# isl-org/Open3D

Hardware: AMD Instinct MI355X
Metric: RGB-D frames/s, TSDF integrate with known poses (configs[1]: touch + activate + integrate into an 8 mm / 16^3 VoxelBlockGrid); the ICP + integrate + ray-cast loop (configs[2]) is in loop_frames_per_s (its first tracked frame untimed as warm-up; the whole run in loop_frames_per_s_with_first_frame) (higher is better)
Workload: dtype f32; 1 GPU; block_count=50000, frames_per_launch=12, active_blocks=5745

## Files before the change

include/o3d_mi355x_host.h:

```cpp
#ifndef O3D_MI355X_HOST_H_
#define O3D_MI355X_HOST_H_

#include "o3d_mi355x.h"

#ifdef __cplusplus
extern "C" {
#endif

typedef struct {
    double relative_fitness;
    double relative_rmse;
    int max_iteration;
} o3dmi_icp_criteria_t;

typedef struct {
    double transformation[16];
    double inlier_rmse;
    double fitness;
    int converged;
    int num_iterations;
    int64_t num_correspondences;
} o3dmi_registration_result_t;

typedef void (*o3dmi_icp_callback_t)(int64_t iteration_index,
// ... 488 lines not shown
                          int frames_per_launch, int slice_rank,
                          int slice_world, void* segment_out_dev,
                          o3dmi_stream_t stream);
int o3dmi_vbg_integrate_frames_sliced(
        o3dmi_vbg_t* g, int n_frames, const void* const* depth_devs,
        int depth_rows, int depth_cols, const void* const* color_devs,
        int color_rows, int color_cols, int input_dtype,
        const double* depth_intrinsic, const double* color_intrinsic,
        const double* extrinsics, float depth_scale, float depth_max,
        float trunc_voxel_multiplier, int frames_per_launch,
        const void* const* gathered_devs, o3dmi_stream_t stream);
int o3dmi_vbg_sliced_stats(const o3dmi_vbg_t* g, int64_t* chunks,
                           int64_t* reapplied, int* capacity,
                           int* table_slots);

int o3dmi_vbg_profile_begin(o3dmi_vbg_t* g, int max_launches, int stride);
int o3dmi_vbg_profile_end(o3dmi_vbg_t* g, o3dmi_stream_t stream,
                          double* integrate_ms, int64_t* launches,
                          int64_t* block_frames, int64_t* frames);
int64_t o3dmi_vbg_profile_distinct_blocks(const o3dmi_vbg_t* g);
int o3dmi_vbg_division_forms(float voxel_size, float trunc_voxel_multiplier,
                             int wait);
int64_t o3dmi_vbg_step_form_launches(int form);
int64_t o3dmi_vbg_profile_launches(const o3dmi_vbg_t* g, int64_t capacity,
                                   float* ms, int32_t* block_frames,
                                   int32_t* distinct_blocks,
                                   int32_t* map_size);

int o3dmi_vbg_ray_cast(o3dmi_vbg_t* g, const int32_t* block_coords_dev,
                       int64_t m, const double* intrinsic,
                       const double* extrinsic, int width, int height,
                       float* range_map_dev, float* out_depth,
                       float* out_vertex, float* out_color, float* out_normal,
                       int64_t* out_index, uint8_t* out_mask, float* out_ratio,
                       float* out_ratio_dx, float* out_ratio_dy,
                       float* out_ratio_dz, float depth_scale, float depth_min,
                       float depth_max, float weight_threshold,
                       float trunc_voxel_multiplier, int range_map_down_factor,
                       o3dmi_stream_t stream);

int o3dmi_vbg_ray_cast_sharded(
        o3dmi_vbg_t* g, const int32_t* block_coords_dev, int64_t m,
        const double* intrinsic, const double* extrinsic, int width, int height,
        float* range_map_dev, float* out_depth, float* out_vertex,
        float* out_color, float* out_normal, float depth_scale, float depth_min,
        float depth_max, float weight_threshold, float trunc_voxel_multiplier,
// ... 153 lines not shown
```

open3d_amd/_lib.py:

```python
import ctypes as C
import os

_HERE = os.path.dirname(os.path.abspath(__file__))
SO_PATH = os.environ.get("O3DMI_LIB") or os.path.join(
    _HERE, "lib", "libo3d_mi355x.so")

OK = 0
F32, F64, U16, U8, I32, I64 = 0, 1, 2, 3, 4, 5
I8, I16, U32, U64, BOOL = 6, 7, 8, 9, 10

_vp = C.c_void_p
_i64 = C.c_int64
_i32 = C.c_int
_f = C.c_float
_d = C.c_double
_dp = C.POINTER(C.c_double)

PROTOTYPES = {
    "o3dmi_abi_version": (_i32, []),
    "o3dmi_status_string": (C.c_char_p, [_i32]),
    "o3dmi_last_error": (C.c_char_p, []),
    "o3dmi_device_info": (_i32, [C.c_char_p, C.c_size_t, C.POINTER(_i32),
                                 C.POINTER(_i64)]),
    "o3dmi_release_cached_memory": (_i32, []),
# ... 431 lines not shown
    "o3dmi_npz_get": (_i32, [_vp, C.c_char_p, C.POINTER(_i32),
                             C.POINTER(_i32), C.POINTER(_i64),
                             C.POINTER(_vp)]),
    "o3dmi_npz_write": (_i32, [_vp, C.c_char_p]),
    "o3dmi_npz_read": (_i32, [C.c_char_p, C.POINTER(_vp)]),
    "o3dmi_vbg_export_blocks": (_i32, [_vp, _i64, _vp, C.POINTER(_vp),
                                       C.POINTER(_i64), _vp]),
    "o3dmi_vbg_merge_blocks": (_i32, [_vp, _vp, C.POINTER(_vp), _i64, _vp]),
    "o3dmi_vbg_save": (_i32, [_vp, C.c_char_p, _vp]),
    "o3dmi_vbg_load": (_i32, [C.c_char_p, _vp, C.POINTER(_vp)]),
    "o3dmi_vbg_attribute_count": (_i32, [_vp]),
    "o3dmi_vbg_attribute_name": (C.c_char_p, [_vp, _i32]),
    "o3dmi_vbg_voxel_size": (_f, [_vp]),
    "o3dmi_vbg_block_resolution": (_i64, [_vp]),
    "o3dmi_vbg_ray_cast": (
        _i32, [_vp, _vp, _i64, _dp, _dp, _i32, _i32, _vp] + [_vp] * 10 +
        [_f, _f, _f, _f, _f, _i32, _vp]),
    "o3dmi_vbg_ray_cast_sharded": (
        _i32, [_vp, _vp, _i64, _dp, _dp, _i32, _i32, _vp] + [_vp] * 4 +
        [_f, _f, _f, _f, _f, _i32, _vp]),
    "o3dmi_vbg_profile_distinct_blocks": (_i64, [_vp]),
    "o3dmi_vbg_division_forms": (_i32, [_f, _f, _i32]),
    "o3dmi_vbg_step_form_launches": (_i64, [_i32]),
    "o3dmi_vbg_profile_launches": (_i64, [_vp, _i64, _vp, _vp, _vp, _vp]),
    "o3dmi_rccl_available": (_i32, []),
    "o3dmi_rccl_unique_id": (_i32, [_vp]),
    "o3dmi_comm_create_rccl": (_i32, [_vp, _i32, _i32, C.POINTER(_vp)]),
    "o3dmi_comm_adopt_rccl": (_i32, [_vp, C.POINTER(_vp)]),
    "o3dmi_comm_create_custom": (_i32, [_vp, _vp, _i32, _i32,
                                        C.POINTER(_vp)]),
    "o3dmi_comm_destroy": (_i32, [_vp]),
    "o3dmi_comm_rank": (_i32, [_vp]),
    "o3dmi_preload": (_i32, []),
    "o3dmi_comm_world": (_i32, [_vp]),
    "o3dmi_comm_rccl_ranks": (_i32, [_vp]),
    "o3dmi_set_comm": (_i32, [_vp]),
    "o3dmi_set_rccl_comm": (_i32, [_vp]),
    "o3dmi_comm_allreduce_sum_f64": (_i32, [_vp, _vp, _i64, _vp]),
    "o3dmi_comm_allgather": (_i32, [_vp, _vp, _vp, _i64, _vp]),
    "o3dmi_comm_alltoallv": (_i32, [_vp, _vp, C.POINTER(_i64),
                                    C.POINTER(_i64), _vp, C.POINTER(_i64),
                                    C.POINTER(_i64), _vp]),
    "o3dmi_vbg_merge_frame_sharded": (_i32, [_vp, _vp, _vp]),
    "o3dmi_vbg_allgather_owned_blocks": (_i32, [_vp, _vp, _vp]),
})

# ... 62 lines not shown
```

open3d_amd/csrc/common.h:

```cpp
#pragma once

#include <hip/hip_runtime.h>

#include <cstdint>
#include <cstdio>
#include <cstring>
#include <string>
#include <vector>

#include "o3d_mi355x.h"

namespace o3dmi {

void SetLastError(const std::string& msg);

int PoolAlloc(void** out, size_t bytes);
void PoolFree(void* p);

struct PoolScratch {
    hipStream_t s;
    std::vector<void*> blocks;
    explicit PoolScratch(hipStream_t st) : s(st) {}
    PoolScratch(const PoolScratch&) = delete;
    PoolScratch& operator=(const PoolScratch&) = delete;
// ... 250 lines not shown
                                   __HIP_MEMORY_SCOPE_AGENT) == in_class - 1) {
            __hip_atomic_store(&tickets[1 + cls], 0, __ATOMIC_RELAXED,
                               __HIP_MEMORY_SCOPE_AGENT);
            last = __hip_atomic_fetch_add(&tickets[0], 1, __ATOMIC_RELAXED,
                                          __HIP_MEMORY_SCOPE_AGENT) ==
                   classes - 1;
            if (last)
                __hip_atomic_store(&tickets[0], 0, __ATOMIC_RELAXED,
                                   __HIP_MEMORY_SCOPE_AGENT);
        }
        s_last_arrival = last;
    }
    __syncthreads();
    return s_last_arrival != 0;
}

constexpr int kTouchBits = 16;
__device__ __forceinline__ unsigned long long* TouchWord(const HashView& hv,
                                                         unsigned slot,
                                                         int plane) {
    return hv.slot_touch + ((size_t)plane * ((size_t)hv.mask + 1) + slot);
}
__device__ __forceinline__ bool TouchSlot(const HashView& hv, unsigned slot,
                                          unsigned long long stamp, int bit,
                                          int plane = 0) {
    unsigned long long* w = TouchWord(hv, slot, plane);
    unsigned long long cur = *w;
    while (true) {
        const bool fresh = (cur >> kTouchBits) != stamp;
        const unsigned long long want =
                fresh ? ((stamp << kTouchBits) | (1ull << bit))
                      : (cur | (1ull << bit));
        if (want == cur) return false;
        const unsigned long long old = atomicCAS(w, cur, want);
        if (old == cur) return fresh;
        cur = old;
    }
}


}

struct o3dmi_hash {
    o3dmi::HashView view;
    int64_t capacity = 0;
    int64_t n_slots = 0;
    int n_values = 0;
    int64_t value_dsizes[8] = {0};
    void* value_buffers[8] = {nullptr};
    int* scratch_count = nullptr;
    int* counters_host = nullptr;
};

namespace o3dmi {
int ClearHashAndCounter(o3dmi_hash* h, int* counter_dev, hipStream_t s);
// ... 2 lines not shown
```

open3d_amd/csrc/host/vbg_grid.cpp:

```cpp

#include <cstdlib>
#include <cstring>

#include "vbg.h"

using namespace o3dmi;

namespace {

int EnsureCapacity(o3dmi_vbg* g, int64_t length, o3dmi_stream_t stream) {
    if (g->size_event_pending) {
        O3DMI_HIP_CHECK(hipEventSynchronize(g->size_event));
        g->size_event_pending = false;
        g->size_bound = g->size_host[0];
    }
    int64_t capacity = o3dmi_hash_capacity(g->block_hashmap);
    if (g->size_bound + length <= capacity) {
        g->size_bound += length;
        return O3DMI_OK;
    }
    int64_t size = 0;
    int st = o3dmi_hash_size(g->block_hashmap, stream, &size);
    if (st) return st;
    int64_t new_size = size + length;
// ... 258 lines not shown
            e = hipHostMalloc((void**)&g->size_host, sizeof(int) * 4);
        if (e == hipSuccess)
            e = hipEventCreateWithFlags(&g->size_event, hipEventDisableTiming);
        if (e != hipSuccess) st = O3DMI_ERR_HIP;
    }
    if (st != O3DMI_OK) {
        o3dmi_vbg_destroy(g);
        return st;
    }
    if (block_resolution % 4 == 0)
        (void)PrefetchFastDivision(voxel_size * 8.0f, false);
    *out = g;
    return O3DMI_OK;
}

int o3dmi_vbg_division_forms(float voxel_size, float trunc_voxel_multiplier,
                             int wait) {
    return PrefetchFastDivision(voxel_size * trunc_voxel_multiplier, wait != 0);
}

int64_t o3dmi_vbg_step_form_launches(int form) {
    return (int64_t)StepFormLaunches(form);
}

int o3dmi_vbg_to_device(o3dmi_vbg_t* g, int device, o3dmi_vbg_t** out) {
    O3DMI_REQUIRE(g != nullptr && out != nullptr, "null argument");
    int cur = 0;
    O3DMI_HIP_CHECK(hipGetDevice(&cur));
    o3dmi_hash_t* hm = nullptr;
    int st = o3dmi_hash_to_device(g->block_hashmap, device, &hm);
    if (st) return st;
    auto* n = new o3dmi_vbg();
    n->voxel_size = g->voxel_size;
    n->block_resolution = g->block_resolution;
    n->attr_names = g->attr_names;
    n->attr_dtypes = g->attr_dtypes;
    n->attr_channels = g->attr_channels;
    n->owner_rank = g->owner_rank;
    n->owner_world = g->owner_world;
    n->block_hashmap = hm;
    hipError_t e = hipSetDevice(device);
    if (e == hipSuccess)
        e = hipMalloc((void**)&n->frame_count, sizeof(int32_t) * 4);
    if (e == hipSuccess)
        e = hipHostMalloc((void**)&n->size_host, sizeof(int) * 4);
    if (e == hipSuccess)
// ... 458 lines not shown
```

open3d_amd/csrc/stream_path.h:

```cpp
#pragma once

#include "common.h"

namespace o3dmi {

constexpr int kMaxGroup = 16;
static_assert(kMaxGroup == kTouchBits, "one touch bit per frame of a group");
constexpr int kDefaultGroup = 8;
constexpr int kGroupChunk = 4;

struct alignas(16) FrameBlock {
    int slot, x, y, z;
};

struct alignas(16) ReadyEntry {
    unsigned long long key;
    int block_idx;
    unsigned bits;
};

struct alignas(8) PixelRec {
    float d;
    unsigned rgba;
};
// ... 39 lines not shown
    int64_t list_capacity;
    int grid_hint;
    float* tsdf;
    void* weight;
    void* color;
    int grid_dtype;
    const double* depth_intrinsic;
    int resolution;
    float voxel_size, sdf_trunc, depth_max;
    float depth_scale;
    int* zero_counter;
    int* size_host;
    int status_stamp;
    int* prof_count;
    int* prof_frame_blocks;
    int* prof_map_size;
};

int LaunchFrameStep(o3dmi_hash* block_hash, const FrameFrontArgs* fronts,
                    int n_fronts, const IntegrateStreamArgs* integ,
                    hipStream_t s);

long long StepFormLaunches(int form);

int PrefetchFastDivision(float sdf_trunc, bool wait);

int RecoverOverflow(o3dmi_hash* block_hash, hipStream_t s, int64_t* wanted);

bool PrepTables(const double* depth_intrinsic, const double* color_intrinsic,
                int rows, int cols, int color_rows, int color_cols,
                float depth_scale, int* col, int* row);

int64_t FrustumBlockBound(const double* intrinsic, int rows, int cols,
                          float depth_max, float block_size, int stride);

}
```

open3d_amd/csrc/touch_device.h:

```cpp
#pragma once

#include "common.h"

namespace o3dmi {

template <bool kAllocate>
__device__ __forceinline__ bool InsertKey(const HashView& hv, int x, int y,
                                          int z, unsigned& slot_out,
                                          int overflow_stamp = 0) {
    slot_out = 0;
    if (kAllocate && overflow_stamp != 0 && hv.counters[3] != 0) return false;
    const int claim = ClaimSlot(hv, PackKey(x, y, z), slot_out,
                                !(kAllocate && overflow_stamp != 0));
    if (claim == -1 && kAllocate && overflow_stamp != 0) {
        atomicCAS(&hv.counters[3], 0, overflow_stamp);
        slot_out = 0;
        return false;
    }
    if (claim != 1) return false;
    if (kAllocate) {
        const unsigned h = slot_out;
        int top = atomicAdd(&hv.counters[0], 1);
        if (top >= hv.capacity) {
            if (overflow_stamp != 0) {
// ... 23 lines not shown
    int lane = threadIdx.x & 63;
    bool decided = !valid;
    while (remaining) {
        int first = __ffsll((long long)remaining) - 1;
        unsigned long long kf = __shfl(k, first);
        bool same = valid && (k == kf);
        unsigned long long same_mask = __ballot(same);
        if (same && !decided) {
            leader = (lane == first);
            decided = true;
        }
        remaining &= ~same_mask;
    }
    return leader;
}

struct TouchParams {
    Camera cam;
    int rows, cols, stride;
    int rows_strided, cols_strided;
    float block_size, sdf_trunc, depth_scale, depth_max;
};

template <typename depth_t>
__device__ __forceinline__ bool RayCandidates(const TouchParams& p,
                                              const depth_t* __restrict__ depth,
                                              int workload_idx, int (&xb)[4],
                                              int (&yb)[4], int (&zb)[4]) {
    int y = (workload_idx / p.cols_strided) * p.stride;
    int x = (workload_idx % p.cols_strided) * p.stride;
    float d = (float)depth[(int64_t)y * p.cols + x] / p.depth_scale;
    if (!(d > 0 && d < p.depth_max)) return false;

    float x_c, y_c, z_c, x_g, y_g, z_g;
    p.cam.Unproject((float)x, (float)y, 1.0f, x_c, y_c, z_c);
    p.cam.RigidTransform(x_c, y_c, z_c, x_g, y_g, z_g);
    float x_o = p.cam.e[0][3], y_o = p.cam.e[1][3], z_o = p.cam.e[2][3];
    float x_d = x_g - x_o, y_d = y_g - y_o, z_d = z_g - z_o;

    const float t_min = fmaxf(d - p.sdf_trunc, 0.0f);
    const float t_max = fminf(d + p.sdf_trunc, p.depth_max);
    const float t_step = (t_max - t_min) / 3;
    float t = t_min;
#pragma unroll
    for (int step = 0; step < 4; ++step) {
        xb[step] = (int)floorf((x_o + t * x_d) / p.block_size);
        yb[step] = (int)floorf((y_o + t * y_d) / p.block_size);
        zb[step] = (int)floorf((z_o + t * z_d) / p.block_size);
        t += t_step;
    }
    return true;
}


inline TouchParams MakeTouchParams(const double* intrinsic, const double* extrinsic,
                            int rows, int cols, int stride, int resolution,
                            float voxel_size, float sdf_trunc,
                            float depth_scale, float depth_max) {
    TouchParams p;
    double pose[16];
    InverseTransformation(extrinsic, pose);
    p.cam = Camera::Make(intrinsic, pose, 1.0f);
    p.rows = rows;
    p.cols = cols;
    p.stride = stride;
    p.rows_strided = rows / stride;
    p.cols_strided = cols / stride;
    p.block_size = voxel_size * resolution;
    p.sdf_trunc = sdf_trunc;
    p.depth_scale = depth_scale;
    p.depth_max = depth_max;
    return p;
}

// ... 3 lines not shown
```

open3d_amd/csrc/vbg_stream.hip:

```cpp

#include <cmath>

#include "common.h"
#include "preload.h"
#include <atomic>
#include <cmath>
#include <cstdio>
#include <cstdlib>
#include <cstring>
#include <map>
#include <mutex>
#include <string>
#include <type_traits>

#include "integrate_checks.h"
#include "stream_path.h"
#include "sliced_path.h"
#include "touch_device.h"

#ifndef O3DMI_ABLATE_GATHER
#define O3DMI_ABLATE_GATHER 0
#endif

namespace o3dmi {
namespace {

template <typename T, int N, int A>
struct alignas(A) Vec {
    T v[N];
};

__device__ __forceinline__ float DivByConst(float a, float b, float y) {
    const float q0 = a * y;
    const float r = __builtin_fmaf(-b, q0, a);
    return __builtin_fmaf(r, y, q0);
}
__device__ __forceinline__ float RecordDepth(float d, float depth_max) {
    return (!(d <= 0) && !(d > depth_max)) ? d : -__builtin_inff();
}

struct PrepParams {
    Camera color_cam;
    int color_rows, color_cols;
    bool with_color;
};

constexpr int kTileKeys = 2048;

struct FrontShared {
    TouchParams p;
    PrepParams pp;
    const int* col_lut;
    const int* row_lut;
    bool depth_div_short;
    bool prep_identity;
    float inv_depth_scale;
    FrameBlock* list;
    int64_t list_capacity;
    int* out_count;
    ReadyEntry* ready;
    int* tickets;
    int* touch_status;
    int n_touch_total;
    unsigned long long group_stamp;
    int touch_plane;
    int n_touch_wg, n_prep_wg;
};
inline bool SameIntrinsics(const Camera& a, const Camera& b) {
    return a.fx == b.fx && a.fy == b.fy && a.cx == b.cx && a.cy == b.cy &&
           a.scale == b.scale;
}
inline bool SameGroup(const FrontShared& a, const FrontShared& b) {
    return SameIntrinsics(a.p.cam, b.p.cam) && a.p.rows == b.p.rows &&
           a.p.cols == b.p.cols && a.p.stride == b.p.stride &&
           a.p.rows_strided == b.p.rows_strided &&
           a.p.cols_strided == b.p.cols_strided &&
           a.p.block_size == b.p.block_size &&
           a.p.sdf_trunc == b.p.sdf_trunc &&
           a.p.depth_scale == b.p.depth_scale &&
           a.p.depth_max == b.p.depth_max &&
           SameIntrinsics(a.pp.color_cam, b.pp.color_cam) &&
           a.pp.color_rows == b.pp.color_rows &&
           a.pp.color_cols == b.pp.color_cols &&
           a.pp.with_color == b.pp.with_color && a.col_lut == b.col_lut &&
           a.row_lut == b.row_lut && a.depth_div_short == b.depth_div_short &&
           a.prep_identity == b.prep_identity &&
           a.inv_depth_scale == b.inv_depth_scale && a.list == b.list &&
           a.list_capacity == b.list_capacity && a.out_count == b.out_count &&
           a.ready == b.ready && a.tickets == b.tickets &&
           a.touch_status == b.touch_status &&
           a.n_touch_total == b.n_touch_total &&
           a.group_stamp == b.group_stamp && a.touch_plane == b.touch_plane &&
           a.n_touch_wg == b.n_touch_wg && a.n_prep_wg == b.n_prep_wg;
}
struct FrontFrame {
    float pose[3][4];
    const uint16_t* depth;
    const uint8_t* color;
    PixelRec* recs;
    int group_bit;
};

struct FrontParams {
    TouchParams p;
    PrepParams pp;
    const uint16_t* depth;
    const uint8_t* color;
    const int* col_lut;
    const int* row_lut;
    bool depth_div_short;
    bool prep_identity;
    float inv_depth_scale;
    PixelRec* recs;
    FrameBlock* list;
    int64_t list_capacity;
    int* out_count;
    ReadyEntry* ready;
    int* tickets;
    int* touch_status;
    int n_touch_total;
    unsigned long long group_stamp;
    int group_bit;
    int touch_plane;
    int n_touch_wg, n_prep_wg;
    __device__ __forceinline__ FrontParams(const FrontShared& s,
                                           const FrontFrame& f)
        : p(s.p), pp(s.pp), depth(f.depth), color(f.color),
          col_lut(s.col_lut), row_lut(s.row_lut),
          depth_div_short(s.depth_div_short), prep_identity(s.prep_identity),
          inv_depth_scale(s.inv_depth_scale), recs(f.recs), list(s.list),
          list_capacity(s.list_capacity), out_count(s.out_count),
          ready(s.ready), tickets(s.tickets), touch_status(s.touch_status),
          n_touch_total(s.n_touch_total),
          group_stamp(s.group_stamp), group_bit(f.group_bit),
          touch_plane(s.touch_plane), n_touch_wg(s.n_touch_wg),
          n_prep_wg(s.n_prep_wg) {
#pragma unroll
        for (int i = 0; i < 3; ++i)
#pragma unroll
            for (int j = 0; j < 4; ++j) p.cam.e[i][j] = f.pose[i][j];
    }
};

__device__ __forceinline__ void FrontRole(const HashView& hv,
                                          const FrontParams& fp, int wg) {
    const TouchParams& p = fp.p;
    const PrepParams& pp = fp.pp;
    const uint16_t* __restrict__ depth = fp.depth;
    const uint8_t* __restrict__ color = fp.color;
    PixelRec* __restrict__ recs = fp.recs;
    FrameBlock* __restrict__ list = fp.list;
    const int n_touch_wg = fp.n_touch_wg;
    if (wg < n_touch_wg) {
        __shared__ unsigned long long tile_keys[kTileKeys];
        for (int e = threadIdx.x; e < kTileKeys; e += blockDim.x)
            tile_keys[e] = kEmptyKey;
        __syncthreads();
        const int tiles_x = (p.cols_strided + 15) >> 4;
        const int ty = wg / tiles_x, tx = wg - ty * tiles_x;
        const int rx = tx * 16 + (threadIdx.x & 15);
        const int ry = ty * 16 + (threadIdx.x >> 4);
        if (rx < p.cols_strided && ry < p.rows_strided) {
            int xb[4], yb[4], zb[4];
            if (RayCandidates(p, depth, ry * p.cols_strided + rx, xb, yb, zb)) {
#pragma unroll
                for (int s = 0; s < 4; ++s) {
                    if (s > 0 && xb[s] == xb[s - 1] && yb[s] == yb[s - 1] &&
                        zb[s] == zb[s - 1])
                        continue;
                    if (!KeyInRange(xb[s], yb[s], zb[s])) {
                        atomicOr(&hv.counters[1], kErrKeyRange);
                        continue;
                    }
                    const unsigned long long k = PackKey(xb[s], yb[s], zb[s]);
                    if (!hv.Owns(k)) continue;
                    unsigned h = HashKey(k) & (kTileKeys - 1);
                    while (true) {
                        unsigned long long cur = tile_keys[h];
                        if (cur == k) break;
                        if (cur == kEmptyKey) {
                            cur = atomicCAS(&tile_keys[h], kEmptyKey, k);
                            if (cur == kEmptyKey || cur == k) break;
                        }
                        h = (h + 1) & (kTileKeys - 1);
                    }
                }
            }
        }
        __syncthreads();
        for (int e = threadIdx.x; e < kTileKeys; e += blockDim.x) {
            const unsigned long long k = tile_keys[e];
            if (k == kEmptyKey) continue;
            const int x = (int)((k >> 42) & 0x1FFFFFull) - kKeyBias;
            const int y = (int)((k >> 21) & 0x1FFFFFull) - kKeyBias;
            const int z = (int)(k & 0x1FFFFFull) - kKeyBias;
            unsigned slot;
            InsertKey<true>(hv, x, y, z, slot, (int)fp.group_stamp);
            if (TouchSlot(hv, slot, fp.group_stamp, fp.group_bit,
                          fp.touch_plane)) {
                int o = atomicAdd(fp.out_count, 1);
                if (o < fp.list_capacity) {
                    unsigned long long* e =
                            reinterpret_cast<unsigned long long*>(&list[o]);
                    __hip_atomic_store(
                            e, (unsigned long long)(unsigned)slot |
                                       ((unsigned long long)(unsigned)x << 32),
                            __ATOMIC_RELAXED, __HIP_MEMORY_SCOPE_AGENT);
                    __hip_atomic_store(
                            e + 1, (unsigned long long)(unsigned)y |
                                           ((unsigned long long)(unsigned)z << 32),
                            __ATOMIC_RELAXED, __HIP_MEMORY_SCOPE_AGENT);
                } else {
                    atomicOr(&hv.counters[1], kErrCapacity);
                }
            }
        }
        if (fp.ready &&
            LastArrival(fp.tickets, fp.group_bit * n_touch_wg + wg,
                        fp.n_touch_total)) {
            int n = __hip_atomic_load(fp.out_count, __ATOMIC_RELAXED,
                                      __HIP_MEMORY_SCOPE_AGENT);
            if (n > fp.list_capacity) n = (int)fp.list_capacity;
            const int overflow = __hip_atomic_load(
                    &hv.counters[3], __ATOMIC_RELAXED, __HIP_MEMORY_SCOPE_AGENT);
            if (overflow != 0) {
                n = 0;
                if (threadIdx.x == 0)
                    __hip_atomic_store(fp.out_count, 0, __ATOMIC_RELAXED,
                                       __HIP_MEMORY_SCOPE_AGENT);
            }
            if (threadIdx.x == 0 && fp.touch_status) {
                const int top = __hip_atomic_load(&hv.counters[0],
                                                  __ATOMIC_RELAXED,
                                                  __HIP_MEMORY_SCOPE_AGENT);
                fp.touch_status[0] = top < hv.capacity ? top : hv.capacity;
                fp.touch_status[1] = overflow;
                fp.touch_status[2] = n;
                __hip_atomic_store(&fp.touch_status[3], (int)fp.group_stamp,
                                   __ATOMIC_RELEASE, __HIP_MEMORY_SCOPE_SYSTEM);
            }
            const auto make_entry = [&](int i) -> ReadyEntry {
                const unsigned long long* e =
// ... 39 lines not shown
                }
#pragma unroll
                for (int k = 0; k < kPerLane; ++k)
                    if (pc[k] >= 0) atomicAdd(&s_bins[pc[k]], 1);
                __syncthreads();
                if (threadIdx.x == 0) {
                    int run = 0;
                    for (int b = kTouchBits; b >= 0; --b) {
                        const int c = s_bins[b];
                        s_bins[b] = run;
                        run += c;
                    }
                }
                __syncthreads();
#pragma unroll
                for (int k = 0; k < kPerLane; ++k)
                    if (pc[k] >= 0)
                        fp.ready[atomicAdd(&s_bins[pc[k]], 1)] = mine[k];
            } else {
                for (int i = threadIdx.x; i < n; i += blockDim.x)
                    fp.ready[i] = make_entry(i);
            }
        }
        return;
    }
    const int n_px = p.rows * p.cols;
    const int n_wg = fp.n_prep_wg;
    if (wg == n_touch_wg && threadIdx.x == 0) {
        PixelRec r;
        r.d = -__builtin_inff();
        r.rgba = 0u;
        recs[n_px] = r;
    }
    if (fp.col_lut && fp.prep_identity) {
        const int n_groups = n_px >> 2;
        const int gstep = n_wg * blockDim.x;
        constexpr int kG = 4;
        for (int g0 = (wg - n_touch_wg) * blockDim.x + threadIdx.x;
             g0 < n_groups; g0 += kG * gstep) {
            uint2 dq[kG];
            unsigned cw[kG][3];
#pragma unroll
            for (int k = 0; k < kG; ++k) {
                const int g = g0 + k * gstep;
                const int gc = g < n_groups ? g : n_groups - 1;
                dq[k] = *reinterpret_cast<const uint2*>(depth + 4 * (int64_t)gc);
                if (pp.with_color) {
                    const unsigned* c = reinterpret_cast<const unsigned*>(
                            color + 12 * (int64_t)gc);
                    cw[k][0] = c[0];
                    cw[k][1] = c[1];
                    cw[k][2] = c[2];
                }
            }
#pragma unroll
            for (int k = 0; k < kG; ++k) {
                const int g = g0 + k * gstep;
                if (g >= n_groups) continue;
                const unsigned dv[4] = {dq[k].x & 0xffffu, dq[k].x >> 16,
                                        dq[k].y & 0xffffu, dq[k].y >> 16};
                unsigned rgba[4] = {0u, 0u, 0u, 0u};
// ... 12 lines not shown
                    const float df = (float)dv[j];
                    const float d =
                            fp.depth_div_short
                                    ? DivByConst(df, p.depth_scale,
                                                 fp.inv_depth_scale)
                                    : df / p.depth_scale;
                    w[2 * j] = __float_as_uint(RecordDepth(d, p.depth_max));
                    w[2 * j + 1] = rgba[j];
                }
                o[0] = make_uint4(w[0], w[1], w[2], w[3]);
                o[1] = make_uint4(w[4], w[5], w[6], w[7]);
                uint4* dst = reinterpret_cast<uint4*>(recs + 4 * (int64_t)g);
                dst[0] = o[0];
                dst[1] = o[1];
            }
        }
        return;
    }
    if (fp.col_lut) {
        const int* __restrict__ col_lut = fp.col_lut;
        const int* __restrict__ row_lut = fp.row_lut;
        const int step = n_wg * blockDim.x;
        const int step_v = step / p.cols, step_u = step - step_v * p.cols;
        for (int first = (wg - n_touch_wg) * blockDim.x + threadIdx.x;
             first < n_px; first += 4 * step) {
            int idx[4], uc[4], vc[4];
            float df[4];
#pragma unroll
            for (int k = 0; k < 4; ++k) {
                const int i = first + k * step;
                idx[k] = i < n_px ? i : n_px - 1;
                df[k] = (float)depth[idx[k]];
            }
            if (pp.with_color) {
                int vi = first / p.cols;
                int ui = first - vi * p.cols;
#pragma unroll
                for (int k = 0; k < 4; ++k) {
                    uc[k] = col_lut[ui];
                    vc[k] = row_lut[vi < p.rows ? vi : p.rows - 1];
                    ui += step_u;
                    vi += step_v;
                    if (ui >= p.cols) {
                        ui -= p.cols;
                        ++vi;
                    }
                }
// ... 13 lines not shown
                    c2[k] = in[2];
                }
#pragma unroll
                for (int k = 0; k < 4; ++k)
                    rgba[k] = (uc[k] | vc[k]) >= 0
                                      ? (c0[k] | (c1[k] << 8) | (c2[k] << 16) |
                                         (1u << 24))
                                      : 0u;
            }
#pragma unroll
            for (int k = 0; k < 4; ++k) {
                PixelRec r;
                r.d = RecordDepth(fp.depth_div_short
                                          ? DivByConst(df[k], p.depth_scale,
                                                       fp.inv_depth_scale)
                                          : df[k] / p.depth_scale,
                                  p.depth_max);
                r.rgba = rgba[k];
                if (first + k * step < n_px) recs[idx[k]] = r;
            }
        }
        return;
    }
    for (int i = (wg - n_touch_wg) * blockDim.x + threadIdx.x; i < n_px;
         i += n_wg * blockDim.x) {
        const int vi = i / p.cols;
        const int ui = i - vi * p.cols;
        PixelRec r;
        r.d = RecordDepth((float)depth[i] / p.depth_scale, p.depth_max);
        r.rgba = 0u;
        if (pp.with_color) {
            float x, y, z, uf, vf;
            p.cam.Unproject((float)ui, (float)vi, 1.0f, x, y, z);
            pp.color_cam.Project(x, y, z, uf, vf);
            if (InBoundary2D(uf, vf, pp.color_rows, pp.color_cols)) {
                int uc = (int)roundf(uf);
                int vc = (int)roundf(vf);
                const uint8_t* in =
                        color + ((int64_t)vc * pp.color_cols + uc) * 3;
                r.rgba = (unsigned)in[0] | ((unsigned)in[1] << 8) |
                         ((unsigned)in[2] << 16) | (1u << 24);
            }
        }
        recs[i] = r;
    }
}

// ... 625 lines not shown
                int n_set = 0;
#pragma unroll
                for (int w = 0; w < kChunkWords; ++w)
                    n_set += __popc((unsigned)__builtin_amdgcn_readlane(
                            (int)long_bits, w));
                unsigned long long* o = ip.prof_items + (b * parts + part) * 4;
                o[0] = item_t0;
                o[1] = wall_clock64();
                o[2] = ((unsigned long long)n_set << 32) |
                       (unsigned)__builtin_amdgcn_s_getreg((31 << 11) | 4);
                o[3] = ((unsigned long long)(unsigned)xcd << 32) | (unsigned)wg;
            }
        }
    }
    if (frame_blocks) atomicAdd(ip.prof_frame_blocks, frame_blocks);
}

struct StepParams {
    HashView hv;
    FrontShared fshared;
    FrontFrame front[kMaxGroup];
    IntegParams integ;
    int n_fronts;
    int front_wg;
};
static_assert(sizeof(StepParams) <= 4096, "kernel arguments are limited to 4 KB");


#ifndef O3DMI_RAW_CHUNK
#define O3DMI_RAW_CHUNK 4
#endif
#ifndef O3DMI_RAW_WAVES
#define O3DMI_RAW_WAVES 5
#endif
constexpr int kRawChunk = O3DMI_RAW_CHUNK;
template <typename weight_t, typename color_t, bool kColor, int kDiv,
          bool kProven>
__device__ __forceinline__ void FrameStep(const StepParams& sp) {
    const int b = (int)blockIdx.x;
    const int n_front_wg = sp.n_fronts * sp.front_wg;
    if (b < n_front_wg) {
        const int f = b / sp.front_wg;
        const FrontParams fp(sp.fshared, sp.front[f]);
        FrontRole(sp.hv, fp, b - f * sp.front_wg);
    } else {
        IntegrateRoleWide<weight_t, color_t, kColor, kDiv, kGroupChunk, 1,
                          false, false, kProven>(
                sp.hv, sp.integ, b - n_front_wg, (int)gridDim.x - n_front_wg,
                n_front_wg);
    }
}
template <typename weight_t, typename color_t, bool kColor, int kDiv>
__global__ void __launch_bounds__(256, 7)
FrameStepKernel(StepParams sp) {
    FrameStep<weight_t, color_t, kColor, kDiv, false>(sp);
}
template <typename weight_t, typename color_t, bool kColor, int kDiv>
__global__ void __launch_bounds__(256, 7)
FrameStepKernelProven(StepParams sp) {
    FrameStep<weight_t, color_t, kColor, kDiv, true>(sp);
}

struct ChunkParams {
    HashView hv;
    IntegParams integ;
};
template <typename weight_t, typename color_t, bool kColor, int kDiv,
          bool kRaw>
__global__ void __launch_bounds__(256, kRaw ? O3DMI_RAW_WAVES : 7)
ChunkIntegrateKernel(ChunkParams cp) {
    IntegrateRoleWide<weight_t, color_t, kColor, kDiv,
                      kRaw ? kRawChunk : kGroupChunk, 1, kRaw, true>(
// ... 135 lines not shown
        return 0;
    }
    const int flags = *p.flag_host;
    p.result = flags < 0 ? 0 : DivFormsFromFlags(flags);
    DivProofReport(b, p.result, flags);
    if (p.stream) {
        (void)hipStreamDestroy(p.stream);
        p.stream = nullptr;
    }
    return p.result;
}

int PrefetchFastDivision(float sdf_trunc, bool wait) {
    float y;
    return VerifyFastDivision(sdf_trunc, &y, wait);
}

static void CanonicalPrincipalPoint(Camera& c) {
    if (c.cx == 0.0f) c.cx = 0.0f;
    if (c.cy == 0.0f) c.cy = 0.0f;
}

static std::atomic<long long> g_step_form_launches[3];

long long StepFormLaunches(int form) {
    return form >= 0 && form < 3
                   ? g_step_form_launches[form].load(std::memory_order_relaxed)
                   : -1;
}

int LaunchFrameStep(o3dmi_hash* bh, const FrameFrontArgs* fronts, int n_fronts,
                    const IntegrateStreamArgs* a, hipStream_t s) {
    O3DMI_REQUIRE((n_fronts > 0 && fronts) || a, "nothing to launch");
    O3DMI_REQUIRE(n_fronts >= 0 && n_fronts <= kMaxGroup, "bad group size");
    StepParams sp = {};
    sp.hv = bh->view;
    sp.n_fronts = n_fronts;
    int n_int_wg = 0;
    int grid_dtype = O3DMI_U16;
    bool col = false;
    int fast_div = 0;
    bool proven = false;
    static const double eye4[16] = {1, 0, 0, 0, 0, 1, 0, 0,
                                    0, 0, 1, 0, 0, 0, 0, 1};
    for (int i = 0; i < n_fronts; ++i) {
        const FrameFrontArgs* f = &fronts[i];
// ... 19 lines not shown
        fs.pp.color_cols = f->color_cols;
        fs.pp.with_color = f->color != nullptr;
        fs.col_lut = f->col_lut;
        fs.row_lut = f->col_lut ? f->row_lut : nullptr;
        fs.depth_div_short = f->depth_div_short;
        fs.prep_identity = f->col_lut && f->prep_identity &&
                           (f->cols % 4) == 0 && f->rows == f->color_rows &&
                           f->cols == f->color_cols;
        fs.inv_depth_scale = 1.0f / f->depth_scale;
        fs.list = f->list;
        fs.list_capacity = f->list_capacity;
        fs.out_count = f->count;
        fs.ready = f->ready;
        fs.tickets = f->ready ? f->tickets : nullptr;
        fs.touch_status = f->ready ? f->touch_status : nullptr;
        fs.group_stamp = f->group_stamp;
        fs.touch_plane = f->touch_plane & 1;
        fs.n_touch_wg = f->prepare_only
                                ? 0
                                : ((tp.cols_strided + 15) / 16) *
                                          ((tp.rows_strided + 15) / 16);
        fs.n_prep_wg = (f->rows * f->cols + kBlock * 16 - 1) / (kBlock * 16);
        if (fs.n_prep_wg < 1) fs.n_prep_wg = 1;
        fs.n_touch_total = fs.n_touch_wg * n_fronts;
        if (i == 0) {
            sp.fshared = fs;
            sp.front_wg = fs.n_touch_wg + fs.n_prep_wg;
        } else {
            O3DMI_REQUIRE(SameGroup(sp.fshared, fs),
                          "frames of one launch must share image size, "
                          "intrinsics, scales and their group");
        }
    }
    if (a) {
        O3DMI_REQUIRE(a->resolution % 4 == 0,
                      "frame-stream path needs block_resolution % 4 == 0");
        O3DMI_REQUIRE(a->n_frames >= 1 && a->n_frames <= kMaxGroup,
                      "bad group size");
        IntegParams& ip = sp.integ;
        ip.n_frames = a->n_frames;
        ip.group_stamp = a->group_stamp;
        ip.touch_plane = a->touch_plane & 1;
        bool fold = SdfDivGuardRedundant(a->depth_scale, a->sdf_trunc);
        bool rcp_ok = true;
        for (int f = 0; f < a->n_frames; ++f) {
            const Camera cf = Camera::Make(a->depth_intrinsic, a->extrinsic[f],
                                           a->voxel_size);
            fold = fold && DepthFoldPoseOk(cf.e, a->voxel_size, a->resolution,
                                           a->sdf_trunc);
            rcp_ok = rcp_ok &&
// ... 25 lines not shown
        ip.tsdf = a->tsdf;
        ip.weight = a->weight;
        ip.color = a->color;
        ip.zero_counter = a->zero_counter;
        ip.size_host = a->size_host;
        ip.status_stamp = a->status_stamp;
        ip.prof_count = a->prof_count;
        ip.prof_frame_blocks = a->prof_frame_blocks;
        ip.prof_map_size = a->prof_map_size;
        const int n_quads =
                (a->resolution * a->resolution * a->resolution) >> 1;
        const int parts = (n_quads + 255) >> 8;
        int64_t g = ((int64_t)a->grid_hint + (a->grid_hint >> 2) + 64) * parts;
        const int64_t g_max = (int64_t)kCUs * 32;
        if (g > g_max) g = g_max;
        if (g < kCUs) g = kCUs;
        n_int_wg = (int)g;
        grid_dtype = a->grid_dtype;
        col = a->with_color && a->color != nullptr;
        proven = fast_div == 2 && rcp_ok;
        g_step_form_launches[proven ? 2 : (fast_div == 2 ? 1 : 0)].fetch_add(
                1, std::memory_order_relaxed);
    }
    dim3 grid((unsigned)(n_fronts * sp.front_wg + n_int_wg)), block(256);
#define O3DMI_LAUNCH_STEP(WT, VT, COLOR)                                      \
    do {                                                                      \
        if (proven)                                                           \
            hipLaunchKernelGGL((FrameStepKernelProven<WT, VT, COLOR, 2>),     \
                               grid, block, 0, s, sp);                        \
        else if (fast_div == 2)                                               \
            hipLaunchKernelGGL((FrameStepKernel<WT, VT, COLOR, 2>), grid,     \
                               block, 0, s, sp);                              \
        else                                                                  \
            hipLaunchKernelGGL((FrameStepKernel<WT, VT, COLOR, 0>), grid,     \
                               block, 0, s, sp);                              \
    } while (0)
    if (grid_dtype == O3DMI_U16) {
        if (col) O3DMI_LAUNCH_STEP(uint16_t, uint16_t, true);
        else O3DMI_LAUNCH_STEP(uint16_t, uint16_t, false);
    } else {
        if (col) O3DMI_LAUNCH_STEP(float, float, true);
        else O3DMI_LAUNCH_STEP(float, float, false);
    }
#undef O3DMI_LAUNCH_STEP
    O3DMI_HIP_CHECK(hipGetLastError());
    return O3DMI_OK;
}
// ... 127 lines not shown
```

open3d_amd/csrc/vbg_touch.hip:

```cpp

#include "common.h"
#include "preload.h"
#include <map>
#include <utility>

#include "touch_device.h"

namespace o3dmi {
namespace {

template <typename depth_t>
__global__ void DepthTouchKernel(HashView hv, TouchParams p,
                                 const depth_t* __restrict__ depth,
                                 int* __restrict__ out_coords,
                                 int64_t out_capacity,
                                 int* __restrict__ out_count) {
    int n = p.rows_strided * p.cols_strided;
    int n_padded = ((n + 63) / 64) * 64;
    for (int w = blockIdx.x * blockDim.x + threadIdx.x; w < n_padded;
         w += gridDim.x * blockDim.x) {
        int xb[4], yb[4], zb[4];
        bool valid = (w < n) && RayCandidates(p, depth, w, xb, yb, zb);
#pragma unroll
        for (int s = 0; s < 4; ++s) {
// ... 32 lines not shown
                                    int* __restrict__ out_count,
                                    int frame_stamp) {
    int n = p.rows_strided * p.cols_strided;
    int n_padded = ((n + 63) / 64) * 64;
    for (int w = blockIdx.x * blockDim.x + threadIdx.x; w < n_padded;
         w += gridDim.x * blockDim.x) {
        int xb[4], yb[4], zb[4];
        bool valid = (w < n) && RayCandidates(p, depth, w, xb, yb, zb);
#pragma unroll
        for (int s = 0; s < 4; ++s) {
            bool ok = valid;
            if (ok && s > 0 && xb[s] == xb[s - 1] && yb[s] == yb[s - 1] &&
                zb[s] == zb[s - 1])
                ok = false;
            if (ok && !KeyInRange(xb[s], yb[s], zb[s])) {
                atomicOr(&hv.counters[1], kErrKeyRange);
                ok = false;
            }
            unsigned long long k = ok ? PackKey(xb[s], yb[s], zb[s]) : 0ull;
            if (ok && !hv.Owns(k)) ok = false;
            if (WaveLeaderForKey(k, ok)) {
                unsigned slot;
                InsertKey<true>(hv, xb[s], yb[s], zb[s], slot);
                if (TouchSlot(hv, slot, (unsigned long long)frame_stamp, 0)) {
                    int o = atomicAdd(out_count, 1);
                    if (o < out_capacity) out_slots[o] = (int)slot;
                    else atomicOr(&hv.counters[1], kErrCapacity);
                }
            }
        }
    }
}

__global__ void SlotsToIndicesKernel(HashView hv, int* __restrict__ io,
                                     const int* __restrict__ count,
                                     int64_t capacity) {
    int64_t n = *count;
    if (n > capacity) n = capacity;
    for (int64_t i = blockIdx.x * (int64_t)blockDim.x + threadIdx.x; i < n;
         i += (int64_t)gridDim.x * blockDim.x)
        io[i] = hv.slot_vals[io[i]];
}

__global__ void PointCloudTouchKernel(HashView hv,
                                      const float* __restrict__ pcd, int64_t n,
                                      float block_size, float sdf_trunc,
                                      int* __restrict__ out_coords,
// ... 496 lines not shown
```

Before: 174,300 frames/s.

## Touch all frames of a launch in one shared tile set per workgroup

```diff
diff --git a/include/o3d_mi355x_host.h b/include/o3d_mi355x_host.h
--- a/include/o3d_mi355x_host.h
+++ b/include/o3d_mi355x_host.h
@@ -534,6 +534,7 @@
 int o3dmi_vbg_division_forms(float voxel_size, float trunc_voxel_multiplier,
                              int wait);
 int64_t o3dmi_vbg_step_form_launches(int form);
+int32_t o3dmi_vbg_front_tile_key_limit(void);
 int64_t o3dmi_vbg_profile_launches(const o3dmi_vbg_t* g, int64_t capacity,
                                    float* ms, int32_t* block_frames,
                                    int32_t* distinct_blocks,
diff --git a/open3d_amd/_lib.py b/open3d_amd/_lib.py
--- a/open3d_amd/_lib.py
+++ b/open3d_amd/_lib.py
@@ -477,6 +477,7 @@
     "o3dmi_vbg_profile_distinct_blocks": (_i64, [_vp]),
     "o3dmi_vbg_division_forms": (_i32, [_f, _f, _i32]),
     "o3dmi_vbg_step_form_launches": (_i64, [_i32]),
+    "o3dmi_vbg_front_tile_key_limit": (_i32, []),
     "o3dmi_vbg_profile_launches": (_i64, [_vp, _i64, _vp, _vp, _vp, _vp]),
     "o3dmi_rccl_available": (_i32, []),
     "o3dmi_rccl_unique_id": (_i32, [_vp]),
diff --git a/open3d_amd/csrc/common.h b/open3d_amd/csrc/common.h
--- a/open3d_amd/csrc/common.h
+++ b/open3d_amd/csrc/common.h
@@ -296,15 +296,15 @@
     return hv.slot_touch + ((size_t)plane * ((size_t)hv.mask + 1) + slot);
 }
 __device__ __forceinline__ bool TouchSlot(const HashView& hv, unsigned slot,
-                                          unsigned long long stamp, int bit,
+                                          unsigned long long stamp,
+                                          unsigned long long bits,
                                           int plane = 0) {
     unsigned long long* w = TouchWord(hv, slot, plane);
     unsigned long long cur = *w;
     while (true) {
         const bool fresh = (cur >> kTouchBits) != stamp;
         const unsigned long long want =
-                fresh ? ((stamp << kTouchBits) | (1ull << bit))
-                      : (cur | (1ull << bit));
+                fresh ? ((stamp << kTouchBits) | bits) : (cur | bits);
         if (want == cur) return false;
         const unsigned long long old = atomicCAS(w, cur, want);
         if (old == cur) return fresh;
diff --git a/open3d_amd/csrc/host/vbg_grid.cpp b/open3d_amd/csrc/host/vbg_grid.cpp
--- a/open3d_amd/csrc/host/vbg_grid.cpp
+++ b/open3d_amd/csrc/host/vbg_grid.cpp
@@ -304,6 +304,8 @@
 int64_t o3dmi_vbg_step_form_launches(int form) {
     return (int64_t)StepFormLaunches(form);
 }
+
+int32_t o3dmi_vbg_front_tile_key_limit(void) { return FrontTileKeyLimit(); }
 
 int o3dmi_vbg_to_device(o3dmi_vbg_t* g, int device, o3dmi_vbg_t** out) {
     O3DMI_REQUIRE(g != nullptr && out != nullptr, "null argument");
diff --git a/open3d_amd/csrc/stream_path.h b/open3d_amd/csrc/stream_path.h
--- a/open3d_amd/csrc/stream_path.h
+++ b/open3d_amd/csrc/stream_path.h
@@ -85,6 +85,7 @@
                     hipStream_t s);
 
 long long StepFormLaunches(int form);
+int FrontTileKeyLimit();
 
 int PrefetchFastDivision(float sdf_trunc, bool wait);
 
diff --git a/open3d_amd/csrc/touch_device.h b/open3d_amd/csrc/touch_device.h
--- a/open3d_amd/csrc/touch_device.h
+++ b/open3d_amd/csrc/touch_device.h
@@ -69,14 +69,11 @@
     float block_size, sdf_trunc, depth_scale, depth_max;
 };
 
-template <typename depth_t>
-__device__ __forceinline__ bool RayCandidates(const TouchParams& p,
-                                              const depth_t* __restrict__ depth,
-                                              int workload_idx, int (&xb)[4],
-                                              int (&yb)[4], int (&zb)[4]) {
-    int y = (workload_idx / p.cols_strided) * p.stride;
-    int x = (workload_idx % p.cols_strided) * p.stride;
-    float d = (float)depth[(int64_t)y * p.cols + x] / p.depth_scale;
+__device__ __forceinline__ bool RayCandidatesOfDepth(const TouchParams& p,
+                                                     int x, int y, float raw,
+                                                     int (&xb)[4], int (&yb)[4],
+                                                     int (&zb)[4]) {
+    float d = raw / p.depth_scale;
     if (!(d > 0 && d < p.depth_max)) return false;
 
     float x_c, y_c, z_c, x_g, y_g, z_g;
@@ -97,6 +94,17 @@
         t += t_step;
     }
     return true;
+}
+
+template <typename depth_t>
+__device__ __forceinline__ bool RayCandidates(const TouchParams& p,
+                                              const depth_t* __restrict__ depth,
+                                              int workload_idx, int (&xb)[4],
+                                              int (&yb)[4], int (&zb)[4]) {
+    int y = (workload_idx / p.cols_strided) * p.stride;
+    int x = (workload_idx % p.cols_strided) * p.stride;
+    return RayCandidatesOfDepth(p, x, y, (float)depth[(int64_t)y * p.cols + x],
+                                xb, yb, zb);
 }
 
 
diff --git a/open3d_amd/csrc/vbg_stream.hip b/open3d_amd/csrc/vbg_stream.hip
--- a/open3d_amd/csrc/vbg_stream.hip
+++ b/open3d_amd/csrc/vbg_stream.hip
@@ -46,6 +46,12 @@
 };
 
 constexpr int kTileKeys = 2048;
+constexpr int kTileKeyLimit = kTileKeys - kTileKeys / 32;
+constexpr int kTileDense = 1024;
+static_assert(kTileKeyLimit < kTileKeys && kTileKeys / 2 <= kTileDense &&
+                      4 * 256 <= kTileKeyLimit,
+              "the tile set must keep an empty slot, hold one frame's keys, "
+              "and half of it must fit the dense list");
 
 struct FrontShared {
     TouchParams p;
@@ -61,7 +67,6 @@
     ReadyEntry* ready;
     int* tickets;
     int* touch_status;
-    int n_touch_total;
     unsigned long long group_stamp;
     int touch_plane;
     int n_touch_wg, n_prep_wg;
@@ -89,7 +94,6 @@
            a.list_capacity == b.list_capacity && a.out_count == b.out_count &&
            a.ready == b.ready && a.tickets == b.tickets &&
            a.touch_status == b.touch_status &&
-           a.n_touch_total == b.n_touch_total &&
            a.group_stamp == b.group_stamp && a.touch_plane == b.touch_plane &&
            a.n_touch_wg == b.n_touch_wg && a.n_prep_wg == b.n_prep_wg;
 }
@@ -101,7 +105,7 @@
     int group_bit;
 };
 
-struct FrontParams {
+struct PrepFrameParams {
     TouchParams p;
     PrepParams pp;
     const uint16_t* depth;
@@ -112,112 +116,188 @@
     bool prep_identity;
     float inv_depth_scale;
     PixelRec* recs;
-    FrameBlock* list;
-    int64_t list_capacity;
-    int* out_count;
-    ReadyEntry* ready;
-    int* tickets;
-    int* touch_status;
-    int n_touch_total;
-    unsigned long long group_stamp;
-    int group_bit;
-    int touch_plane;
-    int n_touch_wg, n_prep_wg;
-    __device__ __forceinline__ FrontParams(const FrontShared& s,
-                                           const FrontFrame& f)
+    int n_prep_wg;
+    __device__ __forceinline__ PrepFrameParams(const FrontShared& s,
+                                               const FrontFrame& f)
         : p(s.p), pp(s.pp), depth(f.depth), color(f.color),
           col_lut(s.col_lut), row_lut(s.row_lut),
           depth_div_short(s.depth_div_short), prep_identity(s.prep_identity),
-          inv_depth_scale(s.inv_depth_scale), recs(f.recs), list(s.list),
-          list_capacity(s.list_capacity), out_count(s.out_count),
-          ready(s.ready), tickets(s.tickets), touch_status(s.touch_status),
-          n_touch_total(s.n_touch_total),
-          group_stamp(s.group_stamp), group_bit(f.group_bit),
-          touch_plane(s.touch_plane), n_touch_wg(s.n_touch_wg),
-          n_prep_wg(s.n_prep_wg) {
-#pragma unroll
-        for (int i = 0; i < 3; ++i)
-#pragma unroll
-            for (int j = 0; j < 4; ++j) p.cam.e[i][j] = f.pose[i][j];
-    }
+          inv_depth_scale(s.inv_depth_scale), recs(f.recs),
+          n_prep_wg(s.n_prep_wg) {}
 };
 
-__device__ __forceinline__ void FrontRole(const HashView& hv,
-                                          const FrontParams& fp, int wg) {
-    const TouchParams& p = fp.p;
-    const PrepParams& pp = fp.pp;
-    const uint16_t* __restrict__ depth = fp.depth;
-    const uint8_t* __restrict__ color = fp.color;
-    PixelRec* __restrict__ recs = fp.recs;
+struct TileSet {
+    unsigned long long keys[kTileKeys];
+    unsigned masks[kTileKeys / 2];
+    unsigned short dense[kTileDense];
+    int frame_keys[3];
+    int pos[2];
+};
+
+__device__ __forceinline__ void FlushTileSet(const HashView& hv,
+                                             const FrontShared& fs,
+                                             TileSet& ts, int count, int& pass,
+                                             bool last) {
+    if (count == 0) return;
+    const int tid = (int)threadIdx.x;
+    const int lane = tid & 63;
+    const int span = count <= kTileDense ? kTileKeys : kTileKeys / 2;
+    for (int base = 0; base < kTileKeys; base += span) {
+        int* pos = &ts.pos[pass & 1];
+        unsigned occ = 0;
+        int total = 0;
+#pragma unroll
+        for (int j = 0; j < kTileKeys / 256; ++j) {
+            if (j * 256 < span) {
+                const bool o = ts.keys[base + j * 256 + tid] != kEmptyKey;
+                occ |= (unsigned)o << j;
+                total += __popcll(__ballot(o));
+            }
+        }
+        int at = 0;
+        if (lane == 0 && total) at = atomicAdd(pos, total);
+        at = __builtin_amdgcn_readfirstlane(at);
+#pragma unroll
+        for (int j = 0; j < kTileKeys / 256; ++j) {
+            if (j * 256 < span) {
+                const bool o = (occ >> j) & 1u;
+                const unsigned long long b = __ballot(o);
+                if (o)
+                    ts.dense[at + __popcll(b & ((1ull << lane) - 1ull))] =
+                            (unsigned short)(base + j * 256 + tid);
+                at += __popcll(b);
+            }
+        }
+        __syncthreads();
+        const int n = *pos;
+        const bool final_pass = last && base + span >= kTileKeys;
+        if (tid == 0) ts.pos[(pass + 1) & 1] = 0;
+        for (int i = tid; i < n; i += (int)blockDim.x) {
+            const unsigned e = ts.dense[i];
+            const unsigned long long k = ts.keys[e];
+            const unsigned sh = (e & 1u) * 16u;
+            const unsigned long long bits = (ts.masks[e >> 1] >> sh) & 0xffffu;
+            if (!final_pass) {
+                ts.keys[e] = kEmptyKey;
+                atomicAnd(&ts.masks[e >> 1], ~(0xffffu << sh));
+            }
+            const int x = (int)((k >> 42) & 0x1FFFFFull) - kKeyBias;
+            const int y = (int)((k >> 21) & 0x1FFFFFull) - kKeyBias;
+            const int z = (int)(k & 0x1FFFFFull) - kKeyBias;
+            unsigned slot;
+            InsertKey<true>(hv, x, y, z, slot, (int)fs.group_stamp);
+            if (TouchSlot(hv, slot, fs.group_stamp, bits, fs.touch_plane)) {
+                int o = atomicAdd(fs.out_count, 1);
+                if (o < fs.list_capacity) {
+                    using u64 = unsigned long long;
+                    u64* le = reinterpret_cast<u64*>(&fs.list[o]);
+                    __hip_atomic_store(le,
+                                       (u64)slot | ((u64)(unsigned)x << 32),
+                                       __ATOMIC_RELAXED,
+                                       __HIP_MEMORY_SCOPE_AGENT);
+                    __hip_atomic_store(le + 1,
+                                       (u64)(unsigned)y |
+                                               ((u64)(unsigned)z << 32),
+                                       __ATOMIC_RELAXED,
+                                       __HIP_MEMORY_SCOPE_AGENT);
+                } else {
+                    atomicOr(&hv.counters[1], kErrCapacity);
+                }
+            }
+        }
+        ++pass;
+        if (!final_pass) __syncthreads();
+    }
+}
+
+__device__ __forceinline__ void TouchRole(const HashView& hv,
+                                          const FrontShared& fp,
+                                          const FrontFrame* fronts,
+                                          int n_fronts, int wg) {
     FrameBlock* __restrict__ list = fp.list;
-    const int n_touch_wg = fp.n_touch_wg;
-    if (wg < n_touch_wg) {
-        __shared__ unsigned long long tile_keys[kTileKeys];
+    {
+        TouchParams p = fp.p;
+        __shared__ TileSet ts;
         for (int e = threadIdx.x; e < kTileKeys; e += blockDim.x)
-            tile_keys[e] = kEmptyKey;
+            ts.keys[e] = kEmptyKey;
+        for (int e = threadIdx.x; e < kTileKeys / 2; e += blockDim.x)
+            ts.masks[e] = 0u;
+        if (threadIdx.x < 3) ts.frame_keys[threadIdx.x] = 0;
+        if (threadIdx.x < 2) ts.pos[threadIdx.x] = 0;
         __syncthreads();
+        __builtin_amdgcn_s_setprio(3);
         const int tiles_x = (p.cols_strided + 15) >> 4;
         const int ty = wg / tiles_x, tx = wg - ty * tiles_x;
         const int rx = tx * 16 + (threadIdx.x & 15);
         const int ry = ty * 16 + (threadIdx.x >> 4);
-        if (rx < p.cols_strided && ry < p.rows_strided) {
+        const bool in_tile = rx < p.cols_strided && ry < p.rows_strided;
+        const int frame_max = 4 * min(16, p.cols_strided - tx * 16) *
+                              min(16, p.rows_strided - ty * 16);
+        const int px = rx * p.stride, py = ry * p.stride;
+        const int64_t pix = in_tile ? (int64_t)py * p.cols + px : 0;
+        const auto raw_depth = [&](int f) -> unsigned {
+            const uint16_t* __restrict__ d =
+                    fronts[f < n_fronts ? f : n_fronts - 1].depth;
+            return in_tile ? (unsigned)d[pix] : 0u;
+        };
+        unsigned d0 = raw_depth(0), d1 = raw_depth(1), d2 = raw_depth(2);
+        int pass = 0;
+        int held = 0;
+        int w = 0;
+#pragma unroll 1
+        for (int f = 0; f < n_fronts; ++f) {
+            const unsigned raw = d0;
+            d0 = d1;
+            d1 = d2;
+            d2 = raw_depth(f + 3);
+            if (f > 0) {
+                __syncthreads();
+                held += ts.frame_keys[w];
+                w = w == 2 ? 0 : w + 1;
+                if (threadIdx.x == 0) ts.frame_keys[w == 2 ? 0 : w + 1] = 0;
+                if (held + frame_max > kTileKeyLimit) {
+                    FlushTileSet(hv, fp, ts, held, pass, false);
+                    held = 0;
+                }
+            }
+            const FrontFrame& ff = fronts[f];
+#pragma unroll
+            for (int i = 0; i < 3; ++i)
+#pragma unroll
+                for (int j = 0; j < 4; ++j) p.cam.e[i][j] = ff.pose[i][j];
+            const unsigned fbit = 1u << ff.group_bit;
             int xb[4], yb[4], zb[4];
-            if (RayCandidates(p, depth, ry * p.cols_strided + rx, xb, yb, zb)) {
-#pragma unroll
-                for (int s = 0; s < 4; ++s) {
-                    if (s > 0 && xb[s] == xb[s - 1] && yb[s] == yb[s - 1] &&
-                        zb[s] == zb[s - 1])
-                        continue;
-                    if (!KeyInRange(xb[s], yb[s], zb[s])) {
-                        atomicOr(&hv.counters[1], kErrKeyRange);
-                        continue;
+            if (!RayCandidatesOfDepth(p, px, py, (float)raw, xb, yb, zb))
+                continue;
+#pragma unroll
+            for (int s = 0; s < 4; ++s) {
+                if (s > 0 && xb[s] == xb[s - 1] && yb[s] == yb[s - 1] &&
+                    zb[s] == zb[s - 1])
+                    continue;
+                if (!KeyInRange(xb[s], yb[s], zb[s])) {
+                    atomicOr(&hv.counters[1], kErrKeyRange);
+                    continue;
+                }
+                const unsigned long long k = PackKey(xb[s], yb[s], zb[s]);
+                if (!hv.Owns(k)) continue;
+                unsigned h = HashKey(k) & (kTileKeys - 1);
+                while (true) {
+                    unsigned long long cur = ts.keys[h];
+                    if (cur == k) break;
+                    if (cur == kEmptyKey) {
+                        cur = atomicCAS(&ts.keys[h], kEmptyKey, k);
+                        if (cur == kEmptyKey) atomicAdd(&ts.frame_keys[w], 1);
+                        if (cur == kEmptyKey || cur == k) break;
                     }
-                    const unsigned long long k = PackKey(xb[s], yb[s], zb[s]);
-                    if (!hv.Owns(k)) continue;
-                    unsigned h = HashKey(k) & (kTileKeys - 1);
-                    while (true) {
-                        unsigned long long cur = tile_keys[h];
-                        if (cur == k) break;
-                        if (cur == kEmptyKey) {
-                            cur = atomicCAS(&tile_keys[h], kEmptyKey, k);
-                            if (cur == kEmptyKey || cur == k) break;
-                        }
-                        h = (h + 1) & (kTileKeys - 1);
-                    }
+                    h = (h + 1) & (kTileKeys - 1);
                 }
+                atomicOr(&ts.masks[h >> 1], fbit << ((h & 1u) * 16u));
             }
         }
         __syncthreads();
-        for (int e = threadIdx.x; e < kTileKeys; e += blockDim.x) {
-            const unsigned long long k = tile_keys[e];
-            if (k == kEmptyKey) continue;
-            const int x = (int)((k >> 42) & 0x1FFFFFull) - kKeyBias;
-            const int y = (int)((k >> 21) & 0x1FFFFFull) - kKeyBias;
-            const int z = (int)(k & 0x1FFFFFull) - kKeyBias;
-            unsigned slot;
-            InsertKey<true>(hv, x, y, z, slot, (int)fp.group_stamp);
-            if (TouchSlot(hv, slot, fp.group_stamp, fp.group_bit,
-                          fp.touch_plane)) {
-                int o = atomicAdd(fp.out_count, 1);
-                if (o < fp.list_capacity) {
-                    unsigned long long* e =
-                            reinterpret_cast<unsigned long long*>(&list[o]);
-                    __hip_atomic_store(
-                            e, (unsigned long long)(unsigned)slot |
-                                       ((unsigned long long)(unsigned)x << 32),
-                            __ATOMIC_RELAXED, __HIP_MEMORY_SCOPE_AGENT);
-                    __hip_atomic_store(
-                            e + 1, (unsigned long long)(unsigned)y |
-                                           ((unsigned long long)(unsigned)z << 32),
-                            __ATOMIC_RELAXED, __HIP_MEMORY_SCOPE_AGENT);
-                } else {
-                    atomicOr(&hv.counters[1], kErrCapacity);
-                }
-            }
-        }
-        if (fp.ready &&
-            LastArrival(fp.tickets, fp.group_bit * n_touch_wg + wg,
-                        fp.n_touch_total)) {
+        held += ts.frame_keys[w];
+        FlushTileSet(hv, fp, ts, held, pass, true);
+        if (fp.ready && LastArrival(fp.tickets, wg, fp.n_touch_wg)) {
             int n = __hip_atomic_load(fp.out_count, __ATOMIC_RELAXED,
                                       __HIP_MEMORY_SCOPE_AGENT);
             if (n > fp.list_capacity) n = (int)fp.list_capacity;
@@ -303,11 +383,18 @@
                     fp.ready[i] = make_entry(i);
             }
         }
-        return;
-    }
+    }
+}
+
+__device__ __forceinline__ void PrepareRole(const PrepFrameParams& fp, int wg) {
+    const TouchParams& p = fp.p;
+    const PrepParams& pp = fp.pp;
+    const uint16_t* __restrict__ depth = fp.depth;
+    const uint8_t* __restrict__ color = fp.color;
+    PixelRec* __restrict__ recs = fp.recs;
     const int n_px = p.rows * p.cols;
     const int n_wg = fp.n_prep_wg;
-    if (wg == n_touch_wg && threadIdx.x == 0) {
+    if (wg == 0 && threadIdx.x == 0) {
         PixelRec r;
         r.d = -__builtin_inff();
         r.rgba = 0u;
@@ -317,7 +404,7 @@
         const int n_groups = n_px >> 2;
         const int gstep = n_wg * blockDim.x;
         constexpr int kG = 4;
-        for (int g0 = (wg - n_touch_wg) * blockDim.x + threadIdx.x;
+        for (int g0 = wg * blockDim.x + threadIdx.x;
              g0 < n_groups; g0 += kG * gstep) {
             uint2 dq[kG];
             unsigned cw[kG][3];
@@ -376,7 +463,7 @@
         const int* __restrict__ row_lut = fp.row_lut;
         const int step = n_wg * blockDim.x;
         const int step_v = step / p.cols, step_u = step - step_v * p.cols;
-        for (int first = (wg - n_touch_wg) * blockDim.x + threadIdx.x;
+        for (int first = wg * blockDim.x + threadIdx.x;
              first < n_px; first += 4 * step) {
             int idx[4], uc[4], vc[4];
             float df[4];
@@ -436,7 +523,7 @@
         }
         return;
     }
-    for (int i = (wg - n_touch_wg) * blockDim.x + threadIdx.x; i < n_px;
+    for (int i = wg * blockDim.x + threadIdx.x; i < n_px;
          i += n_wg * blockDim.x) {
         const int vi = i / p.cols;
         const int ui = i - vi * p.cols;
@@ -1108,7 +1195,7 @@
     FrontFrame front[kMaxGroup];
     IntegParams integ;
     int n_fronts;
-    int front_wg;
+    int n_front_wg;
 };
 static_assert(sizeof(StepParams) <= 4096, "kernel arguments are limited to 4 KB");
 
@@ -1123,17 +1210,43 @@
 template <typename weight_t, typename color_t, bool kColor, int kDiv,
           bool kProven>
 __device__ __forceinline__ void FrameStep(const StepParams& sp) {
+    const int n_front_wg = sp.n_front_wg;
+    const int n_touch_wg = sp.fshared.n_touch_wg;
+    const int n_prep_wg = sp.fshared.n_prep_wg;
+    int t = -1, r = -1, i = -1, n_int = 0;
     const int b = (int)blockIdx.x;
-    const int n_front_wg = sp.n_fronts * sp.front_wg;
-    if (b < n_front_wg) {
-        const int f = b / sp.front_wg;
-        const FrontParams fp(sp.fshared, sp.front[f]);
-        FrontRole(sp.hv, fp, b - f * sp.front_wg);
+    if (b < n_touch_wg) {
+        t = b;
+    } else {
+        const int g = (b - n_touch_wg) >> 3, l = (b - n_touch_wg) & 7;
+        const int n_groups = ((int)gridDim.x - n_touch_wg) >> 3;
+        const int npg = (n_front_wg - n_touch_wg + 7) >> 3;
+        n_int = (n_groups - npg) * 8;
+        int pg = -1, before;
+        if (5 * npg <= n_groups) {
+            before = g / 5 < npg ? g / 5 : npg;
+            if (g % 5 == 4 && g / 5 < npg) pg = g / 5;
+        } else {
+            before = g < npg ? g : npg;
+            if (g < npg) pg = g;
+        }
+        if (pg >= 0) {
+            r = pg * 8 + l;
+            if (r >= n_front_wg - n_touch_wg) return;
+        } else {
+            i = (g - before) * 8 + l;
+        }
+    }
+    if (t >= 0) {
+        TouchRole(sp.hv, sp.fshared, sp.front, sp.n_fronts, t);
+    } else if (r >= 0) {
+        const int f = r / n_prep_wg;
+        const PrepFrameParams fp(sp.fshared, sp.front[f]);
+        PrepareRole(fp, r - f * n_prep_wg);
     } else {
         IntegrateRoleWide<weight_t, color_t, kColor, kDiv, kGroupChunk, 1,
-                          false, false, kProven>(
-                sp.hv, sp.integ, b - n_front_wg, (int)gridDim.x - n_front_wg,
-                n_front_wg);
+                          false, false, kProven>(sp.hv, sp.integ, i, n_int,
+                                                 n_touch_wg);
     }
 }
 template <typename weight_t, typename color_t, bool kColor, int kDiv>
@@ -1315,6 +1428,8 @@
 }
 
 static std::atomic<long long> g_step_form_launches[3];
+
+int FrontTileKeyLimit() { return kTileKeyLimit; }
 
 long long StepFormLaunches(int form) {
     return form >= 0 && form < 3
@@ -1380,10 +1495,9 @@
                                           ((tp.rows_strided + 15) / 16);
         fs.n_prep_wg = (f->rows * f->cols + kBlock * 16 - 1) / (kBlock * 16);
         if (fs.n_prep_wg < 1) fs.n_prep_wg = 1;
-        fs.n_touch_total = fs.n_touch_wg * n_fronts;
         if (i == 0) {
             sp.fshared = fs;
-            sp.front_wg = fs.n_touch_wg + fs.n_prep_wg;
+            sp.n_front_wg = fs.n_touch_wg + n_fronts * fs.n_prep_wg;
         } else {
             O3DMI_REQUIRE(SameGroup(sp.fshared, fs),
                           "frames of one launch must share image size, "
@@ -1455,7 +1569,10 @@
         g_step_form_launches[proven ? 2 : (fast_div == 2 ? 1 : 0)].fetch_add(
                 1, std::memory_order_relaxed);
     }
-    dim3 grid((unsigned)(n_fronts * sp.front_wg + n_int_wg)), block(256);
+    const int n_touch = n_fronts > 0 ? sp.fshared.n_touch_wg : 0;
+    dim3 grid((unsigned)(n_touch + ((sp.n_front_wg - n_touch + 7) & ~7) +
+                         ((n_int_wg + 7) & ~7))),
+            block(256);
 #define O3DMI_LAUNCH_STEP(WT, VT, COLOR)                                      \
     do {                                                                      \
         if (proven)                                                           \
diff --git a/open3d_amd/csrc/vbg_touch.hip b/open3d_amd/csrc/vbg_touch.hip
--- a/open3d_amd/csrc/vbg_touch.hip
+++ b/open3d_amd/csrc/vbg_touch.hip
@@ -78,7 +78,8 @@
             if (WaveLeaderForKey(k, ok)) {
                 unsigned slot;
                 InsertKey<true>(hv, xb[s], yb[s], zb[s], slot);
-                if (TouchSlot(hv, slot, (unsigned long long)frame_stamp, 0)) {
+                if (TouchSlot(hv, slot, (unsigned long long)frame_stamp,
+                              1ull)) {
                     int o = atomicAdd(out_count, 1);
                     if (o < out_capacity) out_slots[o] = (int)slot;
                     else atomicOr(&hv.counters[1], kErrCapacity);
```

Measured after the change: 193,800 frames/s (median of 6 runs). 11.2% higher.
